# winger/genome

Measured on AMD Instinct MI355X. Metric: distinct k-mers/s inserted (k=31, 150bp reads), higher is better.
Workload: dtype u64

## Files before the change

genome_amd/csrc/gk_dist.h:

```cpp
#pragma once

#include <condition_variable>
#include <functional>
#include <memory>
#include <mutex>
#include <string>
#include <thread>
#include <vector>

#include "gk_internal.h"

struct gk_dist;
namespace gk {
enum { XP_SUCCESS = 0 };
enum { XP_INT8 = 0, XP_UINT8 = 1, XP_UINT64 = 5, XP_FLOAT64 = 8 };
enum { XP_SUM = 0, XP_MAX = 2 };
struct Transport {
    int (*group_start)(gk_dist *);
    int (*send)(gk_dist *, const void *, size_t count, int dtype, int peer, hipStream_t);
    int (*recv)(gk_dist *, void *, size_t count, int dtype, int peer, hipStream_t);
    int (*group_end)(gk_dist *);
    int (*all_reduce)(gk_dist *, const void *in, void *out, size_t n, int dtype, int op, hipStream_t);
    int (*all_gather)(gk_dist *, const void *in, void *out, size_t n_per_rank, int dtype, hipStream_t);
    std::string (*error_text)(int code);
    void (*close)(gk_dist *);
};
int dist_create_common(gk_ctx *ctx, int rank, int world, gk_dist **out);
}

struct gk_dist {
    gk_ctx *ctx = nullptr;
    int rank = 0, world = 1;
    const gk::Transport *xport = nullptr;
    void *comm = nullptr;
    std::shared_ptr<void> xstate;
    hipStream_t comm_stream = nullptr;
    static constexpr int NROUTE = 3;
    uint8_t *d_sendbuf[NROUTE] = {nullptr, nullptr, nullptr}, *d_recv[2] = {nullptr, nullptr};
    gk::u64 send_cap[NROUTE] = {0, 0, 0}, recv_records[2] = {0, 0};
    int slot = 0;
    struct Route {
        int k = 0, read_len = 0; const void *records = nullptr; gk::u64 nreads = 0;
        const uint32_t *offsets = nullptr; gk::u64 windows = 0;
        bool settled = false;
        int local_rc = 0;
        std::string local_err;
        uint64_t recs[64] = {}, kmers[64] = {};
        bool exchanged = false;
        int rbuf = 0;
        gk::u64 nrec_in = 0, nkm_in = 0, sent = 0;
        int error = 0;
        std::string error_text;
    };
    Route route[NROUTE];
    uint8_t *d_stage[NROUTE] = {nullptr, nullptr, nullptr};
    uint32_t *d_stage_offs[NROUTE] = {nullptr, nullptr, nullptr};
    gk::u64 stage_bytes[NROUTE] = {0, 0, 0}, stage_offs_bytes[NROUTE] = {0, 0, 0};
    int head = 0, npending = 0;
    gk::u64 nexchanged = 0;
    unsigned long long *d_route_cnt = nullptr;
    unsigned long long *h_route_cnt = nullptr;
    hipEvent_t route_done[NROUTE] = {nullptr, nullptr, nullptr};
    hipEvent_t exch_done[NROUTE] = {nullptr, nullptr, nullptr};
    hipEvent_t join = nullptr;
    unsigned long long *d_cnt = nullptr;
    unsigned long long *h_cnt = nullptr;
    float last_ms[4] = {0, 0, 0, 0};
    gk::u64 classify_queries = 0;
    float last_helper_ms = 0;
    std::thread worker;
    std::mutex wmu;
    std::condition_variable wcv;
    std::function<void()> job;
    bool job_pending = false, job_running = false, quit = false;
    std::vector<void *> garbage;
};
```

genome_amd/csrc/gk_dist.hip:

```cpp
#include <dlfcn.h>
#include <time.h>

#include <algorithm>
#include <condition_variable>
#include <cstring>
#include <deque>
#include <functional>
#include <map>
#include <memory>
#include <mutex>
#include <string>
#include <thread>
#include <vector>

#include "gk_binstream.h"
#include "gk_dist.h"
#include "gk_graph.h"
#include "gk_links.h"
#include "gk_support.h"
#include "gk_tile.h"

using namespace gk;

namespace {
// ... 415 lines not shown
    if (!rrc) rrc = skm_route_finish(ctx, h_rc, route_has_windows(rt), P, d->send_cap[b], rt.recs, rt.kmers);
    for (int attempt = 0; rrc == GK_E_CAPACITY && attempt < 4; attempt++) {
        u64 worst = 0;
        for (int p = 0; p < P; p++) worst = std::max<u64>(worst, rt.recs[p]);
        const u64 want = std::max<u64>(d->send_cap[b] * 2, (worst + worst / 8 + 1024) * P);
        if ((e = hipStreamSynchronize(ctx->copy_stream)) != hipSuccess) { rrc = hip_fail(ctx, e, "gk_dist: re-route"); break; }
        if ((rrc = dist_grow(ctx, &d->d_sendbuf[b], &d->send_cap[b], want, slot)) != GK_OK) break;
        if ((rrc = route_launch(d, b)) != GK_OK) break;
        if ((e = hipStreamSynchronize(ctx->copy_stream)) != hipSuccess) { rrc = hip_fail(ctx, e, "gk_dist: re-route"); break; }
        rrc = skm_route_finish(ctx, h_rc, true, P, d->send_cap[b], rt.recs, rt.kmers);
    }
    if (!rrc && ctx->hook_dist_fail) {
        rrc = fail(ctx, ctx->hook_dist_fail, "injected failure (test_dist_fail_exchange)");
        ctx->hook_dist_fail = 0;
    }
    rt.local_rc = rrc;
    if (rrc) rt.local_err = ctx->err;
    rt.settled = true;
    *ms += (float)(now_ms() - t0);
}

static int dist_exchange(gk_dist *d, int b, float *ms) {
    gk_ctx *ctx = d->ctx;
    gk_dist::Route &rt = d->route[b];
    const int P = d->world, slot = d->slot;
    const double t1 = now_ms();
    hipStream_t cs = d->comm_stream;
    auto give_up = [&](int code, const std::string &text) { rt.error = code; rt.error_text = text; *ms += (float)(now_ms() - t1); return code; };
    auto hip_text = [](hipError_t e, const char *what) { (void)hipGetLastError(); return std::string(what) + ": " + hipGetErrorString(e); };
    const u64 region = d->send_cap[b] / (u64)P;
    u64 sent = 0;
    unsigned long long *h_in = d->h_cnt, *h_out = d->h_cnt + 3 * 64, *d_in = d->d_cnt, *d_out = d->d_cnt + 3 * 64;
    for (int p = 0; p < P; p++) {
        h_in[3 * p] = rt.local_rc ? 0 : rt.recs[p];
        h_in[3 * p + 1] = rt.local_rc ? 0 : rt.kmers[p];
        h_in[3 * p + 2] = rt.local_rc ? (unsigned long long)(-rt.local_rc) : 0ull;
        sent += h_in[3 * p + 1];
    }
    hipError_t e = hipMemcpyAsync(d_in, h_in, 3 * P * 8, hipMemcpyHostToDevice, cs);
    if (e != hipSuccess) return give_up(GK_E_HIP, hip_text(e, "gk_dist: counts upload") + " (before anything was posted: the peers will wait; destroy the communicator)");
    int grc = xGroupStart(d);
    for (int p = 0; p < P && grc == ncclSuccess; p++) {
        grc = xSend(d, d_in + 3 * p, 3, ncclUint64, p, cs);
        if (grc == ncclSuccess) grc = xRecv(d, d_out + 3 * p, 3, ncclUint64, p, cs);
    }
    { const int gend = xGroupEnd(d); if (grc == ncclSuccess) grc = gend; }
    if (grc != ncclSuccess) return give_up(GK_E_COMM, "counts exchange: " + comm_error_text(grc));
    e = hipMemcpyAsync(h_out, d_out, 3 * P * 8, hipMemcpyDeviceToHost, cs);
    if (e == hipSuccess) e = hipStreamSynchronize(cs);
    if (e != hipSuccess) return give_up(GK_E_HIP, hip_text(e, "gk_dist: counts download"));
    u64 nrec_in = 0, nkm_in = 0;
    int bad_rank = -1;
    for (int p = 0; p < P; p++) {
        nrec_in += h_out[3 * p]; nkm_in += h_out[3 * p + 1];
        if (h_out[3 * p + 2] && bad_rank < 0) bad_rank = p;
    }
    if (bad_rank >= 0) {
        std::string text = "rank " + std::to_string(bad_rank) + " could not route its share of this batch (status " + std::to_string(-(long long)h_out[3 * bad_rank + 2]) +
                           "): every rank dropped the batch";
        if (rt.local_rc) text += "; this rank: " + rt.local_err;
        return give_up(GK_E_COMM, text);
    }
    const int rb = (int)(d->nexchanged & 1);
    unsigned long long noroom = 0;
    std::string noroom_text;
    if (nrec_in > d->recv_records[rb] || !d->d_recv[rb]) {
        const u64 want = std::max<u64>(nrec_in + nrec_in / 8, 1024);
        uint8_t *nb = nullptr;
        e = pool_malloc(ctx, &nb, want * (u64)slot + 64);
        if (e == hipSuccess) {
            if (d->d_recv[rb]) { std::lock_guard<std::mutex> lk(d->wmu); d->garbage.push_back(d->d_recv[rb]); }
            d->d_recv[rb] = nb; d->recv_records[rb] = want;
        } else { noroom = 1; noroom_text = hip_text(e, "gk_dist: receive buffer"); }
    }
    unsigned long long *d_flag = d->d_cnt + 6 * 64, *h_flag = d->h_cnt + 6 * 64;
    h_flag[0] = noroom;
    e = hipMemcpyAsync(d_flag, h_flag, 8, hipMemcpyHostToDevice, cs);
    if (e != hipSuccess) return give_up(GK_E_HIP, hip_text(e, "gk_dist: ready flag"));
    grc = xAllReduce(d, d_flag, d_flag + 1, 1, ncclUint64, ncclMax, cs);
    if (grc != ncclSuccess) return give_up(GK_E_COMM, "ready reduction: " + comm_error_text(grc));
    e = hipMemcpyAsync(h_flag + 1, d_flag + 1, 8, hipMemcpyDeviceToHost, cs);
    if (e == hipSuccess) e = hipStreamSynchronize(cs);
    if (e != hipSuccess) return give_up(GK_E_HIP, hip_text(e, "gk_dist: ready flag"));
    if (h_flag[1]) return give_up(GK_E_COMM, "a rank had no room for the records addressed to it: every rank dropped the batch" + (noroom ? "; this rank: " + noroom_text : std::string()));
    grc = xGroupStart(d);
    u64 roff = 0;
    for (int p = 0; p < P && grc == ncclSuccess; p++) {
        if (rt.recs[p]) grc = xSend(d, d->d_sendbuf[b] + (u64)p * region * slot, (size_t)rt.recs[p] * slot, ncclUint8, p, cs);
        if (h_out[3 * p] && grc == ncclSuccess) grc = xRecv(d, d->d_recv[rb] + roff * slot, (size_t)h_out[3 * p] * slot, ncclUint8, p, cs);
        roff += h_out[3 * p];
    }
    { const int gend = xGroupEnd(d); if (grc == ncclSuccess) grc = gend; }
    if (grc != ncclSuccess) return give_up(GK_E_COMM, "record exchange: " + comm_error_text(grc));
    e = hipEventRecord(d->exch_done[b], cs);
    if (e != hipSuccess) return give_up(GK_E_HIP, hip_text(e, "gk_dist: exchange event"));
    rt.exchanged = true; rt.rbuf = rb; rt.nrec_in = nrec_in; rt.nkm_in = nkm_in; rt.sent = sent;
    d->nexchanged++;
    *ms += (float)(now_ms() - t1);
    return GK_OK;
}

int gk_dist_count_routed(gk_dist *d, gk_map *local, uint64_t *occurrences_sent, uint64_t *occurrences_owned) {
    if (int rc = dist_check(d)) return rc;
    gk_ctx *ctx = d->ctx;
    constexpr int NR = gk_dist::NROUTE;
    if (occurrences_sent) *occurrences_sent = 0;
    if (occurrences_owned) *occurrences_owned = 0;
    drain_garbage(d);
    if (!d->npending) return fail(ctx, GK_E_STATE, "gk_dist_count_routed: no route was begun (gk_dist_route_begin)");
    const int b = d->head;
    if (!local || local->ctx != ctx) return fail(ctx, GK_E_INVALID, "gk_dist_count_routed: the local map must live on the handle's context");
    if (local->k != d->route[b].k) return fail(ctx, GK_E_KLEN, "gk_dist_count_routed: the route was begun for another k");
    const double t0 = now_ms();
    float ms_route = 0, ms_exch = 0;
    auto drop_head = [&]() { d->head = (d->head + 1) % NR; d->npending--; };
    if (!d->route[b].exchanged && !d->route[b].error) {
        route_settle(d, b, &ms_route);
        (void)dist_exchange(d, b, &ms_exch);
    }
    bool helping = false;
    float hms = 0;
    if (d->npending >= NR && ctx->hook_dist_ahead != 0) {
        const int b1 = (b + 1) % NR;
        if (!d->route[b1].exchanged && !d->route[b1].error) {
            route_settle(d, b1, &ms_route);
            helper_submit(d, [d, b1, &hms]() { (void)dist_exchange(d, b1, &hms); });
            helping = true;
        }
    }
    struct Join { gk_dist *d; bool on; ~Join() { if (on) helper_wait(d); } } join_helper{d, helping};
    const gk_dist::Route rt = d->route[b];
    drop_head();
    if (rt.error) return fail(ctx, rt.error, "gk_dist_count_routed: " + rt.error_text);
    const double t2 = now_ms();
    GK_HIP(ctx, hipStreamWaitEvent(ctx->stream, d->exch_done[b], 0));
    uint64_t occ = 0;
    if (rt.nrec_in) { if (int rc = gk_map_count_superkmers_dev(local, d->d_recv[rt.rbuf], rt.nrec_in, rt.nkm_in, &occ)) return rc; }
    else GK_HIP(ctx, hipStreamSynchronize(ctx->stream));
    const double t3 = now_ms();
    if (helping) { helper_wait(d); join_helper.on = false; }
    const double t4 = now_ms();
    d->last_ms[0] = ms_route; d->last_ms[1] = ms_exch + (float)(t4 - t3); d->last_ms[2] = (float)(t3 - t2); d->last_ms[3] = (float)(t4 - t0);
    d->last_helper_ms = hms;
    if (occurrences_sent) *occurrences_sent = rt.sent;
    if (occurrences_owned) *occurrences_owned = occ;
    return GK_OK;
}

int gk_dist_count_reads_dev(gk_dist *d, gk_map *local, const void *dev_records, uint64_t nreads, int read_len,
                            uint64_t *occurrences_sent, uint64_t *occurrences_owned) {
    if (int rc = dist_check(d)) return rc;
    if (occurrences_sent) *occurrences_sent = 0;
    if (occurrences_owned) *occurrences_owned = 0;
    if (!local || local->ctx != d->ctx) return fail(d->ctx, GK_E_INVALID, "gk_dist_count_reads_dev: the local map must live on the handle's context");
    if (int rc = gk_dist_route_begin(d, local->k, dev_records, nreads, read_len)) return rc;
    return gk_dist_count_routed(d, local, occurrences_sent, occurrences_owned);
}

int gk_dist_count_reads(gk_dist *d, gk_map *local, const uint8_t *bin, size_t nbytes, uint64_t nreads, uint64_t *occurrences_sent,
                        uint64_t *occurrences_owned) {
    if (int rc = dist_check(d)) return rc;
    gk_ctx *ctx = d->ctx;
    constexpr int NR = gk_dist::NROUTE;
    if (occurrences_sent) *occurrences_sent = 0;
    if (occurrences_owned) *occurrences_owned = 0;
    drain_garbage(d);
    int my_rc = GK_OK;
    std::vector<BinChunk> chunks;
    if (!local || local->ctx != ctx) my_rc = fail(ctx, GK_E_INVALID, "gk_dist_count_reads: the local map must live on the handle's context");
    else if (!bin && nreads) my_rc = fail(ctx, GK_E_INVALID, "gk_dist_count_reads: null stream");
    else if (d->npending) my_rc = fail(ctx, GK_E_STATE, "gk_dist_count_reads: routes begun with gk_dist_route_begin are still waiting");
    else if (!k_supported(local->k)) my_rc = fail(ctx, GK_E_UNSUPPORTED_K, "k=" + std::to_string(local->k) + " unsupported");
    size_t pos = 0;
    u64 r = 0;
    while (!my_rc && r < nreads) {
        int err = 0;
        BinChunk c = map_cut_chunk(local, bin, nbytes, nreads, pos, r, true, &err);
        if (err) {
            my_rc = bin_truncated(ctx, err, c.r_begin + c.offs.size());
            break;
        }
        if (!c.valid) break;
        pos += c.bytes; r += c.reads;
        if (c.uniform && c.first_len >= 0 && !ctx->hook_host_ragged) { c.offs.clear(); c.offs.shrink_to_fit(); }
        else if (c.offs.empty()) {
            const u32 rb = 1 + (u32)(c.first_len + 3) / 4;
            c.offs.resize(c.reads + 1);
            for (u64 i = 0; i <= c.reads; i++) c.offs[i] = (u32)(i * rb);
        }
        chunks.push_back(std::move(c));
// ... 647 lines not shown
```

genome_amd/csrc/gk_internal.h:

```cpp
#pragma once

#include <hip/hip_runtime.h>

#include <initializer_list>
#include <map>
#include <mutex>
#include <string>
#include <unordered_map>
#include <vector>

#include "../../include/genome_amd.h"
#include "gk_device.h"

struct gk_ctx {
    int device = 0;
    hipStream_t stream = nullptr;
    hipEvent_t ev0 = nullptr, ev1 = nullptr;
    hipEvent_t pev[6] = {nullptr, nullptr, nullptr, nullptr, nullptr, nullptr};
    hipEvent_t gev2 = nullptr;
    hipEvent_t gev = nullptr;
    bool copy_other_pending = false;
    hipStream_t copy_stream = nullptr;
    hipEvent_t cev[16] = {};
    hipStream_t aux_stream = nullptr;
// ... 10 lines not shown
    int hook_dist_small_send = 0;
    int hook_target_load_pct = 0;
    int hook_cc_find = 3;
    int hook_dist_fail_classify = 0;
    int hook_dist_fail = 0;
    int hook_dist_ahead = -1;
    int hook_p24_pieces = -1;
    int hook_p45_stripes = -1;
    int hook_graph_load_pct = -1;
    int hook_filter_classic = -1;
    int64_t hook_max_stage = 0;
    int hook_host_prefetch = -1;
    int hook_pairs_host = -1;
    int hook_thread_combine = -1;
    int hook_pairs_small_sets = -1;
    int hook_graph_mbt = -1;
    int hook_graph_mbt_keys = 256;
    int hook_walk_queue = -1;
    int hook_p4_grid = -1;
    int hook_p4_wide = -1;
    int hook_fine_exact = -1;
    int64_t hook_fastq_chunk = 0;
    std::multimap<size_t, void *> pool_free_blocks;
    std::unordered_map<void *, size_t> pool_sizes;
    size_t pool_held = 0, pool_limit = 0;
    size_t pool_live = 0, pool_peak = 0;
    size_t mem_budget = 0;
    uint64_t pool_hits = 0, pool_misses = 0;
    std::recursive_mutex pool_mu;
    int cost_state = 0;
    alignas(8) unsigned char cost_blob[96] = {};
    double measured_copy_tbps = 0, measured_cas_gps = 0;
    double ref_copy_tbps = 5.9, ref_cas_gps = 26.7;
    std::string err;
    int hook_dist_fail_reduce = 0;
    float graph_io_ms[4] = {0, 0, 0, 0};
    int hook_max_grid = 0;
    mutable uint64_t hook_max_grid_uses = 0;
    int64_t hook_contigs_chunk = 0;
    int64_t hook_place_slice = 0;
};
inline uint64_t grid_cap(const gk_ctx *ctx) {
    if (ctx->hook_max_grid <= 0) return (uint64_t)ctx->cu_count * 8;
    ctx->hook_max_grid_uses++;
    return (uint64_t)ctx->hook_max_grid;
}

namespace gk {
struct ReadSrc {
    const uint8_t *rec = nullptr;
    uint64_t nreads = 0;
    const uint32_t *off = nullptr;
    uint32_t stride = 0;
    int group = 64;
    int max_len = 255;
    const uint8_t *host = nullptr;
    size_t host_bytes = 0;
    bool verify_uniform = false;
    hipEvent_t ready = nullptr;
    static ReadSrc fixed(const void *dev_records, uint64_t nreads, int read_len) {
        ReadSrc s;
        s.rec = (const uint8_t *)dev_records;
        s.nreads = nreads;
        s.stride = 1 + (uint32_t)(read_len + 3) / 4;
        s.max_len = read_len;
        return s;
    }
    static ReadSrc framed(const uint8_t *d_rec, const uint32_t *d_off, uint64_t nreads) {
        ReadSrc s;
        s.rec = d_rec;
        s.nreads = nreads;
        s.off = d_off;
        return s;
    }
};
int stage_source(gk_ctx *ctx, const ReadSrc &src);
}

namespace gk {
struct PartScratch;
hipError_t pool_malloc(gk_ctx *ctx, void **p, size_t bytes);
hipError_t pool_free(gk_ctx *ctx, void *p);
void pool_release(gk_ctx *ctx);
size_t mem_available(gk_ctx *ctx);
double graph_table_load(gk_ctx *ctx, int k, uint64_t keys);
template <class T> inline hipError_t pool_malloc(gk_ctx *ctx, T **p, size_t bytes) { return pool_malloc(ctx, (void **)p, bytes); }

struct __attribute__((visibility("hidden"))) DevScratch {
    gk_ctx *ctx;
    std::vector<void *> ptrs;
    hipError_t err = hipSuccess;
    struct Status {
        hipError_t e;
        operator hipError_t() const { return e; }
    };
    explicit DevScratch(gk_ctx *c) : ctx(c) {}
    DevScratch(const DevScratch &) = delete;
    DevScratch &operator=(const DevScratch &) = delete;
    ~DevScratch() { for (void *p : ptrs) (void)pool_free(ctx, p); }
    hipError_t error() const { return err; }
    Status note(hipError_t e) {
        if (err == hipSuccess) err = e;
        return {err};
    }
    template <class T> Status get(T **p, uint64_t n) {
        *p = nullptr;
// ... 156 lines not shown
int map_create_for_graph(gk_ctx *ctx, int k, uint64_t keys, gk_map **out);
void *map_scratch(gk_map *m, size_t bytes);
constexpr int PART_RETRY_DIRECT = 1;
constexpr int PART_OUTGREW = 3;
constexpr int PART_NOT_UNIFORM = 2;
struct PartPlan { bool estimate = false; bool fine_exact = false; bool check_canon = false; double grow_ahead = 1.0; };
int part_count(gk_map *m, PartScratch **pps, const ReadSrc &src, const uint64_t *d_keys, uint64_t nkeys_in, uint64_t nkeys_bound,
               bool from_empty, const PartPlan &plan);
struct P4Form {
    const char *name;
    int W, threads, kpt;
    size_t (*lds)(uint32_t nb2, uint32_t nb1);
    int op_wgs_cap;
    int exact_wgs;
    const void *kernel[2];
    void (*launch[2])(const void *p4args);
    uint32_t chunk_keys() const { return (uint32_t)(threads * kpt); }
};
enum PartSource { PART_SRC_DEVICE = 0, PART_SRC_HOST = 1, PART_SRC_PREFETCHED = 2, PART_SRC_RAGGED = 3, PART_SRC_KEYS = 4 };
struct PartInput {
    int W = 1, lnb1 = 8;
    uint32_t nb2 = 1;
    int source = PART_SRC_DEVICE;
    int max_windows = 0;
    bool from_empty = false, verify_uniform = false;
    bool estimate = false, fine_exact = false;
    bool part_exact = false;
    int p4_wide = -1, p4_direct = -1, p2_wide = -1, p2_sorted = -1, p45_stripes = -1, p24_pieces = -1, p4_grid = -1, max_nb2 = 0;
};
struct PartChoice {
    bool supported;
    bool op1, fine_exact, sync_between, pipelined;
    int pieces, op_stripes, p4_per_cu;
    const char *p2;
    int p2_threads; bool p2_sorted; uint32_t p2_nb1;
    const P4Form *p4_op, *p4_exact;
};
PartChoice part_choose(const PartInput &in);
const P4Form *p4_choose_exact(int W, uint32_t nb2, uint32_t nb1, int p4_wide, int p4_direct);
struct BinChunk {
    size_t begin = 0, bytes = 0;
    uint64_t r_begin = 0, reads = 0, occ = 0;
    int first_len = -1;
    bool uniform = true, unverified = false, valid = false;
    std::vector<uint32_t> offs;
};
BinChunk map_cut_chunk(gk_map *m, const uint8_t *bin, size_t nbytes, uint64_t nreads, size_t pos, uint64_t r, bool walk, int *err);
int map_fire_prefetch(gk_map *m, hipEvent_t after);
int map_count_begin(gk_map *m);
uint64_t map_window_limit(gk_map *m);
int map_count_framed_dev(gk_map *m, const uint8_t *d_rec, const uint32_t *d_off, uint64_t nrec, uint64_t windows, double grow_ahead);
int map_count_end(gk_map *m, uint64_t *occurrences);
int map_ensure_sample(gk_map *m);
int map_make_room(gk_map *m, uint64_t new_distinct, uint64_t size_for, bool from_empty, bool keep_lnb1 = false);
uint64_t part_max_slots(int W);
int ctx_check_format(gk_ctx *ctx);
constexpr int SKM_COUNT_WORDS = 2 * 64 + 1;
int skm_route_launch(gk_ctx *ctx, hipStream_t st, unsigned long long *d_counts, unsigned long long *h_counts, int k, const void *dev_records,
                     uint64_t nreads, int read_len, int P, void *dev_out, uint64_t out_cap_records);
int skm_route_launch(gk_ctx *ctx, hipStream_t st, unsigned long long *d_counts, unsigned long long *h_counts, int k, const void *dev_records,
                     const uint32_t *dev_offsets, uint64_t nreads, uint64_t windows, int P, void *dev_out, uint64_t out_cap_records);
int skm_route_finish(gk_ctx *ctx, const unsigned long long *h_counts, bool launched, int P, uint64_t out_cap_records, uint64_t *rec_counts_host,
                     uint64_t *kmer_counts_host);
inline int lanes_per_read(int max_windows) { return max_windows > 32 ? 64 : max_windows > 16 ? 32 : 16; }
bool part_supported(const gk_map *m);
void part_scratch_free(gk_ctx *ctx, PartScratch *ps);

}

#ifdef GK_TIMERS
#define GK_TIMERS_DEFINE(suffix)                                                                                          \
    static __device__ unsigned long long g_timers[16];                                                                   \
    extern "C" int gk_debug_timers_##suffix(unsigned long long *out16, int reset) {                                      \
        if (hipMemcpyFromSymbol(out16, HIP_SYMBOL(g_timers), sizeof(unsigned long long) * 16) != hipSuccess) return -1;  \
        unsigned long long z[16] = {0};                                                                                  \
        if (reset && hipMemcpyToSymbol(HIP_SYMBOL(g_timers), z, sizeof(z)) != hipSuccess) return -1;                     \
        return 0;                                                                                                        \
    }
#define GK_T0() unsigned long long t_prev = __builtin_amdgcn_s_memrealtime(), t_acc[8] = {0, 0, 0, 0, 0, 0, 0, 0}
#define GK_TARGS_DECL unsigned long long &t_prev, unsigned long long (&t_acc)[8]
#define GK_TARGS t_prev, t_acc
#define GK_TICK(i) do { const unsigned long long t_now = __builtin_amdgcn_s_memrealtime(); t_acc[i] += t_now - t_prev; t_prev = t_now; } while (0)
#define GK_TFLUSH(base) do { if (threadIdx.x == 0) for (int q = 0; q < 8; q++) if (t_acc[q]) atomicAdd(&g_timers[(base) + q], t_acc[q]); } while (0)
#else
#define GK_TIMERS_DEFINE(suffix)
#define GK_T0() do {} while (0)
#define GK_TARGS_DECL int
#define GK_TARGS 0
#define GK_TICK(i) do {} while (0)
#define GK_TFLUSH(base) do {} while (0)
#endif
```

genome_amd/csrc/gk_partition.hip:

```cpp
#include <algorithm>
#include <cmath>
#include <cstdlib>
#include <string>
#include <type_traits>
#include <vector>

#include "gk_internal.h"
#include "gk_tile.h"

using namespace gk;

GK_TIMERS_DEFINE(partition)

static constexpr int PBLOCK = 512;
static constexpr int KEYS_PER_THREAD = 8;
static constexpr int PTILE_READS = 256;
static constexpr int PTILE_WORDS = PTILE_READS * 65 / 4 + 64;
static constexpr int TILE2 = PBLOCK * KEYS_PER_THREAD;
static constexpr u32 MAXB1 = 1u << MAX_LNB1;
static constexpr u32 MAX_NB2 = 4096;
#ifndef GK_MAX_RANGE_CHUNKS
#define GK_MAX_RANGE_CHUNKS 96
#endif
static constexpr u32 MAX_RANGE_CHUNKS = GK_MAX_RANGE_CHUNKS;
// ... 1293 lines not shown
            a.chunk_keys = ch.p4_op->chunk_keys();
        }
        a_last = a;
        return GK_OK;
    }
    int raise_lds_limits() {
        auto raise = [&](const void *kernel, size_t bytes) { return hipFuncSetAttribute(kernel, hipFuncAttributeMaxDynamicSharedMemorySize, (int)std::min(bytes, LDS_BYTES_PER_CU)); };
        for (const P4Form &f : P4_FORMS)
            for (const void *kernel : f.kernel)
                if (f.W == W && kernel) GK_HIP(ctx, raise(kernel, f.lds(MAX_NB2, MAXB1)));
        GK_HIP(ctx, raise(reinterpret_cast<const void *>(&k_part_scatter1_keys<W>), ScatterLds<W>::bytes(MAXB1)));
        GK_HIP(ctx, raise(reinterpret_cast<const void *>(&k_seg_insert<W, Slot<W>>), SEG_LDS));
        if constexpr (W == 1) GK_HIP(ctx, raise(reinterpret_cast<const void *>(&k_seg_insert<1, CSlot>), SEG_LDS));
        ps->lds_attr_set = true;
        return GK_OK;
    }

    void launch_p4(const P4Form *f, bool ranged, const PartArrays &aa, hipStream_t st, int grid, u64 max_units, u32 b_lo, u32 b_hi) {
        m->last_p4 = f->name;
        const P4Args<W> x{st, grid, f->lds(m->nb2, nb1), ps->bufA, t, &aa, max_units, ps->bufB, b_lo, b_hi};
        f->launch[ranged](&x);
    }
    void launch_p4_op(const PartArrays &aa, hipStream_t st, u32 b_lo, u32 b_hi, u64 share) {
        const int grid = (int)std::min<u64>(max_chunks / share + 1, (u64)ctx->cu_count * std::min(ch.p4_per_cu, ch.p4_op->op_wgs_cap));
        launch_p4(ch.p4_op, false, aa, st, grid, max_chunks, b_lo, b_hi);
    }

    int p2_grid(u64 nr) const { return (int)std::min<u64>(std::max<u64>((nr + rs - 1) / rs, 1), (u64)ctx->cu_count * GK_OP_WGS_PER_CU); }
    void launch_p2(const uint8_t *recs, u64 nr) {
        m->last_p2 = ch.p2;
#define GK_P2(NT, SORTED, NB1)                                                                                                                  \
    hipLaunchKernelGGL((k_op_scatter1_reads<W, NT, SORTED, NB1>), dim3(p2_grid(nr)), dim3(NT), 0, ctx->stream, recs, nr, src.stride, m->k, src.group, \
                       rs, src.max_len, src.verify_uniform ? 1 : 0, t, a, sp, m->d_ctr, ps->bufA)
        if (ch.p2_nb1 > 256) { if (ch.p2_sorted) GK_P2(PBLOCK, true, (int)MAXB1); else GK_P2(PBLOCK, false, (int)MAXB1); }
        else if (ch.p2_threads == 1024) { if (ch.p2_sorted) GK_P2(1024, true, 256); else GK_P2(1024, false, 256); }
        else if (ch.p2_sorted) GK_P2(PBLOCK, true, 256);
        else GK_P2(PBLOCK, false, 256);
#undef GK_P2
    }
    int piece_done(int j, int npieces) {
        unsigned long long *tab = ps->piece_tables + (size_t)j * PIECE_WORDS;
        const unsigned long long *prev = j ? ps->piece_tables + (size_t)(j - 1) * PIECE_WORDS + MAXB1 : nullptr;
        hipLaunchKernelGGL(k_part_prefix1_piece, dim3(1), dim3(MAXB1), 0, ctx->stream, a, nb1, prev, tab, tab + MAXB1, tab + 2 * MAXB1);
        PartArrays aj = a;
        aj.l1_from = tab; aj.l1_to = tab + MAXB1; aj.cbase = tab + 2 * MAXB1;
        if (j == npieces - 1) { a_last = aj; have_last = true; return GK_OK; }
        hipEvent_t ev = ctx->cev[8 + j % 8];
        GK_HIP(ctx, hipEventRecord(ev, ctx->stream));
        GK_HIP(ctx, hipStreamWaitEvent(ctx->aux_stream, ev, 0));
        launch_p4_op(aj, ctx->aux_stream, 0u, nb1, (u64)npieces);
        GK_HIP(ctx, hipGetLastError());
        return GK_OK;
    }
    int feed_device() { launch_p2(src.rec, src.nreads); return GK_OK; }
    int feed_device_pieces() {
        const u64 min_piece = (u64)rs * (ctx->hook_p24_pieces > 1 ? 64ull : (u64)ctx->cu_count * GK_OP_WGS_PER_CU * 2);
        const u64 np = std::max<u64>(1, std::min<u64>({(u64)ch.pieces, (u64)MAX_PIECES, src.nreads / std::max<u64>(min_piece, 1)}));
        const u64 sub_reads = ((src.nreads + np - 1) / np + rs - 1) / rs * rs;
        const int npieces = (int)((src.nreads + sub_reads - 1) / sub_reads);
        pieces_run = npieces;
        u64 r0 = 0;
        for (int j = 0; j < npieces; j++, r0 += sub_reads) {
            launch_p2(src.rec + (size_t)r0 * src.stride, std::min<u64>(sub_reads, src.nreads - r0));
            if (int rc = piece_done(j, npieces)) return rc;
        }
        return GK_OK;
    }
    int feed_prefetched() {
        GK_HIP(ctx, hipStreamWaitEvent(ctx->stream, src.ready, 0));
        launch_p2(src.rec, src.nreads);
        return ch.pipelined ? piece_done(0, 1) : GK_OK;
    }
    int feed_host() {
        const u64 min_piece = (u64)rs * 1024;
        u64 piece[8];
        int npieces = 0;
        const u64 sub_reads = std::max<u64>(min_piece, ((src.nreads + 7) / 8 + rs - 1) / rs * rs);
        for (u64 done = 0; done < src.nreads && npieces < 8; done += sub_reads) piece[npieces++] = std::min<u64>(sub_reads, src.nreads - done);
        if (ch.pipelined) pieces_run = npieces;
        u64 r0 = 0;
        for (int j = 0; j < npieces; r0 += piece[j], j++) {
            const u64 nr = piece[j];
            if (!nr) continue;
            const size_t off = (size_t)r0 * src.stride, bytes = (size_t)nr * src.stride;
            hipEvent_t ev = ctx->cev[j % 16];
            if (j == 0) {
                GK_HIP(ctx, hipEventRecord(ev, ctx->stream));
                GK_HIP(ctx, hipStreamWaitEvent(ctx->copy_stream, ev, 0));
            }
            GK_HIP(ctx, hipMemcpyAsync(const_cast<uint8_t *>(src.rec) + off, src.host + off, bytes, hipMemcpyHostToDevice, ctx->copy_stream));
            GK_HIP(ctx, hipEventRecord(ev, ctx->copy_stream));
            GK_HIP(ctx, hipStreamWaitEvent(ctx->stream, ev, 0));
            launch_p2(src.rec + off, nr);
            if (ch.pipelined) { if (int rc = piece_done(j, npieces)) return rc; }
        }
        return GK_OK;
    }
    int feed_exact_reads() {
        if (int rc = stage_source(ctx, src)) return rc;
        const u64 ntiles = (src.nreads + PTILE_READS - 1) / PTILE_READS;
        const int grid = (int)std::min<u64>(std::max<u64>(ntiles, 1), (u64)ctx->cu_count * 4);
        hipLaunchKernelGGL(k_part_hist1_reads<W>, dim3(grid), dim3(PBLOCK), 0, ctx->stream, src.rec, src.nreads, src.off, src.stride, m->k, src.group,
                           src.max_len, t, a.hist1, sp, m->d_ctr);
        hipLaunchKernelGGL(k_part_prefix1, dim3(1), dim3(MAXB1), 0, ctx->stream, a, nb1);
        GK_HIP(ctx, hipEventRecord(ctx->pev[1], ctx->stream));
        hipLaunchKernelGGL(k_part_scatter1_reads<W>, dim3(grid), dim3(PBLOCK), 0, ctx->stream, src.rec, src.nreads, src.off, src.stride, m->k, src.group,
                           src.max_len, t, a.l1_base, a.cursor1, ps->bufA);
        return GK_OK;
    }
    int feed_keys() {
        if (!ch.op1) {
            const int grid = (int)std::min<u64>(std::max<u64>((nkeys_in + BLOCK - 1) / BLOCK, 1), (u64)ctx->cu_count * 8);
            hipLaunchKernelGGL(k_part_hist1_keys<W>, dim3(grid), dim3(BLOCK), 0, ctx->stream, d_keys, nkeys_in, t, a.hist1);
            hipLaunchKernelGGL(k_part_prefix1, dim3(1), dim3(MAXB1), 0, ctx->stream, a, nb1);
        }
        GK_HIP(ctx, hipEventRecord(ctx->pev[1], ctx->stream));
        const int g2 = (int)std::min<u64>(std::max<u64>((nkeys_in + TILE2 - 1) / TILE2, 1), (u64)ctx->cu_count * 4);
        hipLaunchKernelGGL(k_part_scatter1_keys<W>, dim3(g2), dim3(PBLOCK), ScatterLds<W>::bytes(std::max(256u, nb1)), ctx->stream, d_keys, nkeys_in, t, a, ps->bufA, sp);
        return GK_OK;
    }

    int l1_level() {
        GK_HIP(ctx, hipEventRecord(ctx->pev[0], ctx->stream));
        m->last_slot = W == 1 && m->layout == LAYOUT_COUNT ? "count12" : W == 1 ? "slot16" : "slot24";
        m->last_p2 = src.rec ? "exact" : ch.p2;
        int rc;
        if (src.rec && ch.op1) {
            GK_HIP(ctx, hipEventRecord(ctx->pev[1], ctx->stream));
            const u64 by_bytes = ((u64)OP_TILE_WORDS * 4 - 96) / src.stride;
            const u64 max_windows = (u64)std::max(0, src.max_len - m->k + 1);
            rs = (int)std::max<u64>(1, std::min<u64>(by_bytes, (u64)(OP_CAP / W) / max_windows));
            rc = !src.host ? (ch.pipelined ? feed_device_pieces() : feed_device()) : src.ready ? feed_prefetched() : feed_host();
        } else {
            rc = src.rec ? feed_exact_reads() : feed_keys();
        }
        if (rc) return rc;
        if (!ch.pipelined) {
            a.chunk_keys = ch.p4_op->chunk_keys();
            if (ch.op1) hipLaunchKernelGGL(k_part_prefix1, dim3(1), dim3(MAXB1), 0, ctx->stream, a, nb1);
        }
        GK_HIP(ctx, hipGetLastError());
        GK_HIP(ctx, hipEventRecord(ctx->pev[2], ctx->stream));
        return map_fire_prefetch(m, ctx->pev[2]);
    }

    int request_status() {
        GK_HIP(ctx, hipMemcpyAsync(h_st, a.nspill, sizeof(PartStatus), hipMemcpyDeviceToHost, ctx->stream));
        return GK_OK;
    }
    int read_counters(Counters *out) {
        GK_HIP(ctx, hipMemcpyAsync(h_ctr, m->d_ctr, sizeof(Counters), hipMemcpyDeviceToHost, ctx->stream));
        GK_HIP(ctx, hipStreamSynchronize(ctx->stream));
        *out = *h_ctr;
        return GK_OK;
    }
    int give_back(int reason, bool table_touched) {
        if (reason == PART_NOT_UNIFORM) GK_HIP(ctx, hipMemsetAsync(&m->d_ctr->format, 0, sizeof(u32), ctx->stream));
        if (!table_touched) GK_HIP(ctx, hipEventRecord(ctx->pev[5], ctx->stream));
        if (src.rec) {
            unsigned long long occ = occ_before;
            GK_HIP(ctx, hipMemcpy(&m->d_ctr->occurrences, &occ, 8, hipMemcpyHostToDevice));
            m->occ_cached = occ;
        }
        if (table_touched) GK_HIP(ctx, hipMemset(&m->d_ctr->size, 0, 8));
        if (reason == PART_RETRY_DIRECT) m->retries_direct++;
        return reason;
    }

    int between_levels() {
        if (src.verify_uniform && !(src.rec && ch.op1)) return fail(ctx, GK_E_STATE, "unverified host stream reached a path that cannot verify it");
        if (ch.sync_between) {
            Counters c;
            if (int rc = request_status()) return rc;
            if (int rc = read_counters(&c)) return rc;
            if (src.verify_uniform && c.format) return give_back(PART_NOT_UNIFORM, false);
            if (h_st->overflow) return give_back(PART_RETRY_DIRECT, false);
            if (plan.estimate) { if (int rc = size_table_from_sample(c)) return rc; }
        }
        if (!part_supported(m)) {
// ... 152 lines not shown
```

genome_amd/csrc/gk_table.hip:

```cpp
#include <algorithm>
#include <sys/syscall.h>
#include <unistd.h>
#include <cstdio>
#include <cstring>
#include <vector>

#include "gk_binstream.h"
#include "gk_internal.h"
#include "gk_scan.h"
#include "gk_tile.h"

using namespace gk;

namespace gk {
static thread_local std::string tls_err;

void set_error(const gk_ctx *ctx, const std::string &msg) {
    tls_err = msg;
    if (ctx) const_cast<gk_ctx *>(ctx)->err = msg;
}
int fail(const gk_ctx *ctx, int code, const std::string &msg) {
    set_error(ctx, msg);
    return code;
}
// ... 848 lines not shown
int gk_map_k(const gk_map *m) { return m ? m->k : 0; }

int gk_map_set_insert_path(gk_map *m, int path) {
    if (int rc = check_map_lazy(m)) return rc;
    if (path < 0 || path > 2) return fail(m->ctx, GK_E_INVALID, "insert path must be 0 (auto), 1 (direct) or 2 (partitioned)");
    if (path == 2 && !part_supported(m)) return fail(m->ctx, GK_E_INVALID, "table too large for the partitioned path");
    m->insert_path = path;
    return GK_OK;
}

int gk_map_clear(gk_map *m) {
    if (int rc = check_map_lazy(m)) return rc;
    gk_ctx *ctx = m->ctx;
    GK_HIP(ctx, hipMemsetAsync(m->d_ctr, 0, sizeof(Counters), ctx->stream));
    if (m->d_sample && m->sample_dirty) GK_HIP(ctx, hipMemsetAsync(m->d_sample, 0xff, (m->sample_mask + 1) * 8, ctx->stream));
    m->sample_claims_seen = 0;
    m->sample_dirty = false;
    m->est_distinct_last = 0;
    m->pending_clear = true;
    m->layout = LAYOUT_COUNT;
    m->size = 0;
    m->tombstones = 0;
    m->total_occurrences = 0;
    m->dirty = false;
    m->masks_valid = false;
    return GK_OK;
}

int gk_map_size(gk_map *m, uint64_t *n) {
    if (int rc = check_map_lazy(m)) return rc;
    if (!n) return fail(m->ctx, GK_E_INVALID, "gk_map_size: n is NULL");
    *n = m->size;
    return GK_OK;
}

int gk_map_slots(gk_map *m, uint64_t *slots) {
    if (int rc = check_map_lazy(m)) return rc;
    if (!slots) return fail(m->ctx, GK_E_INVALID, "gk_map_slots: slots is NULL");
    *slots = m->capacity;
    return GK_OK;
}

static int add_keys_dev(gk_map *m, const u64 *d_keys, const i32 *d_counts, u64 n, bool verbatim = false);

static int launch_count(gk_map *m, const ReadSrc &src) {
    gk_ctx *ctx = m->ctx;
    u64 ntiles = (src.nreads + TILE_READS - 1) / TILE_READS;
    int grid = (int)std::min<u64>(std::max<u64>(ntiles, 1), (u64)ctx->cu_count * 8);
    if (int rc = stage_source(ctx, src)) return rc;
    GK_HIP(ctx, hipEventRecord(ctx->ev0, ctx->stream));
    GK_BY_SLOT(m, hipLaunchKernelGGL((k_count_reads<W, S>), dim3(grid), dim3(BLOCK), 0, ctx->stream, src.rec, src.nreads, src.off, src.stride, m->k, src.group,
                                     src.max_len, table_of<W, S>(m), m->d_ctr));
    GK_HIP(ctx, hipGetLastError());
    GK_HIP(ctx, hipEventRecord(ctx->ev1, ctx->stream));
    if (int rc = map_sync_counters(m)) return rc;
    float ms = 0.f;
    GK_HIP(ctx, hipEventElapsedTime(&ms, ctx->ev0, ctx->ev1));
    m->last_count_ms += ms;
    m->phase_ms[0] += ms;
    m->direct_launches++;
    return GK_OK;
}

static constexpr size_t GK_MAX_STAGE_DEFAULT = 704u << 20;
static inline size_t max_stage(const gk_ctx *ctx) { return ctx->hook_max_stage > 0 ? (size_t)ctx->hook_max_stage : GK_MAX_STAGE_DEFAULT; }
static int reset_occ_counter(gk_map *m) {
    GK_HIP(m->ctx, hipMemsetAsync(&m->d_ctr->occurrences, 0, sizeof(unsigned long long), m->ctx->stream));
    m->occ_cached = 0;
    return GK_OK;
}
static int read_occ_counter(gk_map *m, uint64_t *occ) {
    *occ = m->occ_cached;
    return GK_OK;
}

struct PathCost {
    double direct_ps = 45.0;
    double p2_ps = 5.0;
    double p3_ps = 2.3;
    double p4_ps = 3.9;
    double p4_ps_per_nb2 = 0.0018;
    double p5_ps = 1.7;
    double stream_tbps = 4.6;
    double fixed_us = 60.0;
};
__global__ __launch_bounds__(256) void k_calib_cas(u64 *arr, u64 mask, u64 n) {
    for (u64 i = (u64)blockIdx.x * 256 + threadIdx.x; i < n; i += (u64)gridDim.x * 256) (void)cas64(&arr[mix64(i) & mask], ~0ull, i);
}
static const PathCost &path_cost(gk_ctx *ctx) {
    static const PathCost REF;
    if (ctx->cost_state == 1) return *reinterpret_cast<const PathCost *>(ctx->cost_blob);
    if (ctx->cost_state == 2) return REF;
    static_assert(sizeof(PathCost) <= sizeof(ctx->cost_blob), "cost blob");
    ctx->cost_state = 2;
    constexpr u64 N16 = (64u << 20) / 16, NCAS = 1u << 23;
    uint4 *a = nullptr, *b = nullptr;
    DevScratch tmp(ctx);
    if (tmp.get(&a, N16) != hipSuccess || tmp.get(&b, N16) != hipSuccess) return REF;
    const int grid = ctx->cu_count * 8;
    float ms_copy = 0, ms_cas = 0;
    hipError_t e = hipMemsetAsync(a, 0xff, N16 * 16, ctx->stream);
    for (int r = 0; r < 3 && e == hipSuccess; r++) {
        if (r == 2) e = hipEventRecord(ctx->ev0, ctx->stream);
        hipLaunchKernelGGL(k_stream_copy, dim3(grid), dim3(256), 0, ctx->stream, a, b, N16);
    }
    if (e == hipSuccess) e = hipEventRecord(ctx->ev1, ctx->stream);
// ... 127 lines not shown
}

static void reset_call_stats(gk_map *m) {
    m->gap_ms = 0.f;
    m->last_count_ms = 0.f;
    m->last_count_occ = 0;
    for (float &x : m->phase_ms) x = 0.f;
}

static int count_fixed_records(gk_map *m, ReadSrc src, u64 nk, u64 windows_total ) {
    const uint8_t *rec = src.rec;
    const u64 nreads = src.nreads;
    u64 done = 0;
    while (done < nreads) {
        const u64 left = nreads - done;
        u64 chunk = std::min<u64>(left, std::max<u64>(1, part_batch_keys(m) / std::max<u64>(nk, 1)));
        u64 bound = windows_total && chunk == nreads ? windows_total : chunk * nk;
        if (!(nk && use_partitioned(m, bound))) {
            chunk = std::min(left, reads_per_launch(m, nk));
            bound = windows_total && chunk == nreads ? windows_total : chunk * nk;
        }
        src.rec = rec + done * src.stride;
        src.nreads = chunk;
        if (int rc = insert_batch(m, src, nullptr, 0, bound, false, (double)left / (double)chunk)) return rc;
        done += chunk;
    }
    return GK_OK;
}

int gk_map_count_reads_dev(gk_map *m, const void *dev_records, uint64_t nreads, int read_len, uint64_t *occurrences) {
    if (int rc = check_map_lazy(m)) return rc;
    gk_ctx *ctx = m->ctx;
    if (occurrences) *occurrences = 0;
    if (!dev_records && nreads) return fail(ctx, GK_E_INVALID, "gk_map_count_reads_dev: null records");
    if (read_len < 0 || read_len > 255) return fail(ctx, GK_E_FORMAT, "read_len must be 0..255 (one length byte per record)");
    reset_call_stats(m);
    if (nreads == 0) return GK_OK;
    ReadSrc src;
    src.rec = (const uint8_t *)dev_records;
    src.nreads = nreads;
    src.stride = 1 + (read_len + 3) / 4;
    src.max_len = read_len;
    const u64 nk = read_len >= m->k ? (u64)(read_len - m->k + 1) : 0;
    if (int rc = reset_occ_counter(m)) return rc;
    if (int rc = count_fixed_records(m, src, nk, 0)) return rc;
    uint64_t occ = 0;
    if (int rc = read_occ_counter(m, &occ)) return rc;
    m->last_count_occ = occ;
    m->total_occurrences += occ;
    if (occurrences) *occurrences = occ;
    return GK_OK;
}

int gk_map_count_superkmers_dev(gk_map *m, const void *dev_records, uint64_t nrecords, uint64_t kmers_total, uint64_t *occurrences) {
    if (int rc = check_map_lazy(m)) return rc;
    gk_ctx *ctx = m->ctx;
    if (occurrences) *occurrences = 0;
    if (!dev_records && nrecords) return fail(ctx, GK_E_INVALID, "gk_map_count_superkmers_dev: null records");
    reset_call_stats(m);
    if (nrecords == 0) return GK_OK;
    ReadSrc src;
    src.rec = (const uint8_t *)dev_records;
    src.nreads = nrecords;
    src.stride = m->k <= 31 ? 16u : 32u;
    src.max_len = (int)(src.stride - 1) * 4;
    const u64 max_run = (u64)(src.max_len - m->k + 1);
    if (kmers_total > nrecords * max_run) return fail(ctx, GK_E_INVALID, "kmers_total exceeds what the records can hold");
    if (int rc = reset_occ_counter(m)) return rc;
    src.group = lanes_per_read(std::min<int>((int)max_run, std::max(8, (m->k - 9) * 3 / 4)));
    const u64 bound = ctx->hook_part_exact ? nrecords * max_run : kmers_total;
    if (part_batch_keys(m) >= bound) {
        if (int rc = insert_batch(m, src, nullptr, 0, bound)) return rc;
    } else {
        if (int rc = count_fixed_records(m, src, max_run, 0)) return rc;
    }
    uint64_t occ = 0;
    if (int rc = read_occ_counter(m, &occ)) return rc;
    m->last_count_occ = occ;
    m->total_occurrences += occ;
    if (occurrences) *occurrences = occ;
    if (occ != kmers_total) return fail(ctx, GK_E_FORMAT, "records held " + std::to_string(occ) + " k-mers, caller announced " + std::to_string(kmers_total));
    return GK_OK;
}

static int stage_reserve(gk_map *m, int slot, size_t bytes) {
    gk_ctx *ctx = m->ctx;
    gk_map::StageSlot &st = m->stage[slot];
    if (st.cap >= bytes) return GK_OK;
    if (st.d) {
        GK_HIP(ctx, hipStreamSynchronize(ctx->copy_stream));
        GK_HIP(ctx, pool_free(ctx, st.d));
    }
    st.d = nullptr; st.cap = 0;
    GK_HIP(ctx, pool_malloc(ctx, &st.d, bytes));
    st.cap = bytes;
    return GK_OK;
}
static int stage_prefetch_arm(gk_map *m, const uint8_t *p, size_t bytes, int in_use) {
    gk_ctx *ctx = m->ctx;
    int slot;
    if (in_use >= 0) slot = 1 - in_use;
    else if (m->stage[0].valid != m->stage[1].valid) slot = m->stage[0].valid ? 1 : 0;
    else slot = 1 - m->stage_last_pf;
    gk_map::StageSlot &st = m->stage[slot];
    st.valid = false; st.armed = false;
    if (int rc = stage_reserve(m, slot, bytes + 64)) return rc;
    if (!st.ev) GK_HIP(ctx, hipEventCreateWithFlags(&st.ev, hipEventDisableTiming));
    st.host = p; st.bytes = bytes; st.armed = true;
    m->stage_last_pf = slot;
    return GK_OK;
}
}
namespace gk {
int map_fire_prefetch(gk_map *m, hipEvent_t after) {
    gk_ctx *ctx = m->ctx;
    for (int sl = 0; sl < 2; sl++) {
        gk_map::StageSlot &st = m->stage[sl];
        if (!st.armed) continue;
        st.armed = false;
        if (after) GK_HIP(ctx, hipStreamWaitEvent(ctx->copy_stream, after, 0));
        GK_HIP(ctx, hipMemcpyAsync(st.d, st.host, st.bytes, hipMemcpyHostToDevice, ctx->copy_stream));
        GK_HIP(ctx, hipEventRecord(st.ev, ctx->copy_stream));
        st.valid = true;
    }
    return GK_OK;
}
}
extern "C" {

int gk_map_prefetch_reads(gk_map *m, const uint8_t *bin, size_t nbytes, uint64_t nreads) {
    if (int rc = check_map_lazy(m)) return rc;
    gk_ctx *ctx = m->ctx;
    if (!bin || !nbytes || !nreads) return fail(ctx, GK_E_INVALID, "gk_map_prefetch_reads: empty stream");
    {
        const size_t rb = 1 + (size_t)(bin[0] + 3) / 4;
// ... 617 lines not shown
```

Baseline: 58.39 billion.

## Skip self-send in record exchange and count own records in place

During the all-to-all record exchange, each rank no longer sends records to itself through the collective. Instead, it passes its own region of the send buffer as a second record span to the counting path, which launches the partition or count kernels once per span. This removes a device-side self copy and the receive-buffer space it used. In exchange, the counting code has to handle two spans, and paths that read only one span now return an error or fall back to two separate count passes.

```diff
diff --git a/genome_amd/csrc/gk_dist.h b/genome_amd/csrc/gk_dist.h
--- a/genome_amd/csrc/gk_dist.h
+++ b/genome_amd/csrc/gk_dist.h
@@ -49,6 +49,7 @@
         bool exchanged = false;
         int rbuf = 0;
         gk::u64 nrec_in = 0, nkm_in = 0, sent = 0;
+        gk::u64 nrec_self = 0, nkm_self = 0;
         int error = 0;
         std::string error_text;
     };
diff --git a/genome_amd/csrc/gk_dist.hip b/genome_amd/csrc/gk_dist.hip
--- a/genome_amd/csrc/gk_dist.hip
+++ b/genome_amd/csrc/gk_dist.hip
@@ -491,7 +491,7 @@
     u64 nrec_in = 0, nkm_in = 0;
     int bad_rank = -1;
     for (int p = 0; p < P; p++) {
-        nrec_in += h_out[3 * p]; nkm_in += h_out[3 * p + 1];
+        if (p != d->rank) { nrec_in += h_out[3 * p]; nkm_in += h_out[3 * p + 1]; }
         if (h_out[3 * p + 2] && bad_rank < 0) bad_rank = p;
     }
     if (bad_rank >= 0) {
@@ -525,6 +525,7 @@
     grc = xGroupStart(d);
     u64 roff = 0;
     for (int p = 0; p < P && grc == ncclSuccess; p++) {
+        if (p == d->rank) continue;
         if (rt.recs[p]) grc = xSend(d, d->d_sendbuf[b] + (u64)p * region * slot, (size_t)rt.recs[p] * slot, ncclUint8, p, cs);
         if (h_out[3 * p] && grc == ncclSuccess) grc = xRecv(d, d->d_recv[rb] + roff * slot, (size_t)h_out[3 * p] * slot, ncclUint8, p, cs);
         roff += h_out[3 * p];
@@ -534,6 +535,7 @@
     e = hipEventRecord(d->exch_done[b], cs);
     if (e != hipSuccess) return give_up(GK_E_HIP, hip_text(e, "gk_dist: exchange event"));
     rt.exchanged = true; rt.rbuf = rb; rt.nrec_in = nrec_in; rt.nkm_in = nkm_in; rt.sent = sent;
+    rt.nrec_self = h_out[3 * d->rank]; rt.nkm_self = h_out[3 * d->rank + 1];
     d->nexchanged++;
     *ms += (float)(now_ms() - t1);
     return GK_OK;
@@ -574,7 +576,10 @@
     const double t2 = now_ms();
     GK_HIP(ctx, hipStreamWaitEvent(ctx->stream, d->exch_done[b], 0));
     uint64_t occ = 0;
-    if (rt.nrec_in) { if (int rc = gk_map_count_superkmers_dev(local, d->d_recv[rt.rbuf], rt.nrec_in, rt.nkm_in, &occ)) return rc; }
+    if (rt.nrec_in + rt.nrec_self) {
+        const uint8_t *own = d->d_sendbuf[b] + (u64)d->rank * (d->send_cap[b] / (u64)d->world) * (u64)d->slot;
+        if (int rc = map_count_superkmers_spans(local, d->d_recv[rt.rbuf], rt.nrec_in, own, rt.nrec_self, rt.nkm_in + rt.nkm_self, &occ)) return rc;
+    }
     else GK_HIP(ctx, hipStreamSynchronize(ctx->stream));
     const double t3 = now_ms();
     if (helping) { helper_wait(d); join_helper.on = false; }
diff --git a/genome_amd/csrc/gk_internal.h b/genome_amd/csrc/gk_internal.h
--- a/genome_amd/csrc/gk_internal.h
+++ b/genome_amd/csrc/gk_internal.h
@@ -86,6 +86,8 @@
     uint64_t nreads = 0;
     const uint32_t *off = nullptr;
     uint32_t stride = 0;
+    const uint8_t *rec2 = nullptr;
+    uint64_t nreads2 = 0;
     int group = 64;
     int max_len = 255;
     const uint8_t *host = nullptr;
@@ -348,6 +350,8 @@
 int map_count_framed_dev(gk_map *m, const uint8_t *d_rec, const uint32_t *d_off, uint64_t nrec, uint64_t windows, double grow_ahead);
 int map_count_end(gk_map *m, uint64_t *occurrences);
 int map_ensure_sample(gk_map *m);
+int map_count_superkmers_spans(gk_map *m, const void *recs, uint64_t nrecs, const void *recs2, uint64_t nrecs2, uint64_t kmers_total,
+                               uint64_t *occurrences);
 int map_make_room(gk_map *m, uint64_t new_distinct, uint64_t size_for, bool from_empty, bool keep_lnb1 = false);
 uint64_t part_max_slots(int W);
 int ctx_check_format(gk_ctx *ctx);
diff --git a/genome_amd/csrc/gk_partition.hip b/genome_amd/csrc/gk_partition.hip
--- a/genome_amd/csrc/gk_partition.hip
+++ b/genome_amd/csrc/gk_partition.hip
@@ -1369,7 +1369,11 @@
         GK_HIP(ctx, hipGetLastError());
         return GK_OK;
     }
-    int feed_device() { launch_p2(src.rec, src.nreads); return GK_OK; }
+    int feed_device() {
+        launch_p2(src.rec, src.nreads);
+        if (src.rec2 && src.nreads2) launch_p2(src.rec2, src.nreads2);
+        return GK_OK;
+    }
     int feed_device_pieces() {
         const u64 min_piece = (u64)rs * (ctx->hook_p24_pieces > 1 ? 64ull : (u64)ctx->cu_count * GK_OP_WGS_PER_CU * 2);
         const u64 np = std::max<u64>(1, std::min<u64>({(u64)ch.pieces, (u64)MAX_PIECES, src.nreads / std::max<u64>(min_piece, 1)}));
@@ -1442,6 +1446,7 @@
         m->last_slot = W == 1 && m->layout == LAYOUT_COUNT ? "count12" : W == 1 ? "slot16" : "slot24";
         m->last_p2 = src.rec ? "exact" : ch.p2;
         int rc;
+        if (src.rec2 && !(ch.op1 && !src.host && !ch.pipelined)) return fail(ctx, GK_E_STATE, "a second record span reached a path that reads one span only");
         if (src.rec && ch.op1) {
             GK_HIP(ctx, hipEventRecord(ctx->pev[1], ctx->stream));
             const u64 by_bytes = ((u64)OP_TILE_WORDS * 4 - 96) / src.stride;
diff --git a/genome_amd/csrc/gk_table.hip b/genome_amd/csrc/gk_table.hip
--- a/genome_amd/csrc/gk_table.hip
+++ b/genome_amd/csrc/gk_table.hip
@@ -924,6 +924,14 @@
     GK_BY_SLOT(m, hipLaunchKernelGGL((k_count_reads<W, S>), dim3(grid), dim3(BLOCK), 0, ctx->stream, src.rec, src.nreads, src.off, src.stride, m->k, src.group,
                                      src.max_len, table_of<W, S>(m), m->d_ctr));
     GK_HIP(ctx, hipGetLastError());
+    if (src.rec2 && src.nreads2) {
+        if (src.off || src.host) return fail(ctx, GK_E_STATE, "a second record span needs a fixed-stride device source");
+        ntiles = (src.nreads2 + TILE_READS - 1) / TILE_READS;
+        grid = (int)std::min<u64>(std::max<u64>(ntiles, 1), (u64)ctx->cu_count * 8);
+        GK_BY_SLOT(m, hipLaunchKernelGGL((k_count_reads<W, S>), dim3(grid), dim3(BLOCK), 0, ctx->stream, src.rec2, src.nreads2, src.off, src.stride, m->k, src.group,
+                                         src.max_len, table_of<W, S>(m), m->d_ctr));
+        GK_HIP(ctx, hipGetLastError());
+    }
     GK_HIP(ctx, hipEventRecord(ctx->ev1, ctx->stream));
     if (int rc = map_sync_counters(m)) return rc;
     float ms = 0.f;
@@ -1157,16 +1165,21 @@
     return GK_OK;
 }
 
-int gk_map_count_superkmers_dev(gk_map *m, const void *dev_records, uint64_t nrecords, uint64_t kmers_total, uint64_t *occurrences) {
+}
+namespace gk {
+int map_count_superkmers_spans(gk_map *m, const void *recs, uint64_t nrecs, const void *recs2, uint64_t nrecs2, uint64_t kmers_total,
+                               uint64_t *occurrences) {
     if (int rc = check_map_lazy(m)) return rc;
     gk_ctx *ctx = m->ctx;
     if (occurrences) *occurrences = 0;
-    if (!dev_records && nrecords) return fail(ctx, GK_E_INVALID, "gk_map_count_superkmers_dev: null records");
+    if ((!recs && nrecs) || (!recs2 && nrecs2)) return fail(ctx, GK_E_INVALID, "gk_map_count_superkmers_dev: null records");
     reset_call_stats(m);
-    if (nrecords == 0) return GK_OK;
+    if (nrecs == 0) { recs = recs2; nrecs = nrecs2; recs2 = nullptr; nrecs2 = 0; }
+    if (nrecs == 0) return GK_OK;
+    const u64 nrecords = nrecs + nrecs2;
     ReadSrc src;
-    src.rec = (const uint8_t *)dev_records;
-    src.nreads = nrecords;
+    src.rec = (const uint8_t *)recs;
+    src.nreads = nrecs;
     src.stride = m->k <= 31 ? 16u : 32u;
     src.max_len = (int)(src.stride - 1) * 4;
     const u64 max_run = (u64)(src.max_len - m->k + 1);
@@ -1174,10 +1187,18 @@
     if (int rc = reset_occ_counter(m)) return rc;
     src.group = lanes_per_read(std::min<int>((int)max_run, std::max(8, (m->k - 9) * 3 / 4)));
     const u64 bound = ctx->hook_part_exact ? nrecords * max_run : kmers_total;
-    if (part_batch_keys(m) >= bound) {
+    const bool both_at_once = !nrecs2 || (!ctx->hook_part_exact && ctx->hook_p24_pieces <= 1);
+    if (part_batch_keys(m) >= bound && both_at_once) {
+        src.rec2 = (const uint8_t *)recs2;
+        src.nreads2 = nrecs2;
         if (int rc = insert_batch(m, src, nullptr, 0, bound)) return rc;
     } else {
         if (int rc = count_fixed_records(m, src, max_run, 0)) return rc;
+        if (nrecs2) {
+            src.rec = (const uint8_t *)recs2;
+            src.nreads = nrecs2;
+            if (int rc = count_fixed_records(m, src, max_run, 0)) return rc;
+        }
     }
     uint64_t occ = 0;
     if (int rc = read_occ_counter(m, &occ)) return rc;
@@ -1186,6 +1207,11 @@
     if (occurrences) *occurrences = occ;
     if (occ != kmers_total) return fail(ctx, GK_E_FORMAT, "records held " + std::to_string(occ) + " k-mers, caller announced " + std::to_string(kmers_total));
     return GK_OK;
+}
+}
+extern "C" {
+int gk_map_count_superkmers_dev(gk_map *m, const void *dev_records, uint64_t nrecords, uint64_t kmers_total, uint64_t *occurrences) {
+    return map_count_superkmers_spans(m, dev_records, nrecords, nullptr, 0, kmers_total, occurrences);
 }
 
 static int stage_reserve(gk_map *m, int slot, size_t bytes) {
```

After: 57.73 billion. -1.1%, worse.
